# GAMES-UChile/mogptk

Hardware: AMD Instinct MI355X
Metric: log-marginal-likelihood+grad evals/sec, MOSM C=4 N=8192; 1/2/4/8 GPU (higher is better)
Workload: dtype f64

## Files before the change

mogptk_amd/csrc/flow.hip:

```cpp
#include "mogp_model.h"
#include <unistd.h>
#include <chrono>
#include <set>

#include <cstdio>
#include <cstdlib>

namespace mogp {

typedef double d4_t __attribute__((ext_vector_type(4)));
typedef double d2_t __attribute__((ext_vector_type(2)));

#define FL_BK 16
#define FL_ROWK 18
#define FL_WTM 4
#define FL_WTN 2
#define FL_NWJ 4
#define FL_NWI 2
#define FL_NT 512
#define FL_COLK (MOGP_TILE + 16)
#define FL_OPER (MOGP_TILE * FL_ROWK)
#define FL_LDS_DOUBLES (2 * 2 * FL_OPER)
#define FL_LDS_BYTES (FL_LDS_DOUBLES * 8 + 16 + 3 * 64 * 4 + 16)
static_assert(MOGP_TILE * FL_ROWK == 16 * FL_COLK, "one LDS operand slot serves both layouts");

#define FL_LDS_BARRIER() asm volatile("s_waitcnt lgkmcnt(0)\n\ts_barrier" ::: "memory")

template <int AKM, int BKM, bool MARK = false>
__device__ __forceinline__ void flow_tile(const double* Ap, const double* Bp, double* Cp, const int64_t ld, const int kt, const bool fresh,
                                          const double alpha, double* gemm_lds, unsigned long long* tr, unsigned* prog, double* const* Cpp, const double* alphap) {
    constexpr int WTM = FL_WTM, WTN = FL_WTN, NWJ = FL_NWJ, NWI = FL_NWI, NT = FL_NT;
    constexpr int TMR = MOGP_TILE, TNC = MOGP_TILE, COLK_A = FL_COLK, COLK_B = FL_COLK, OPER_A = FL_OPER, OPER_B = FL_OPER;
    constexpr int EPT_A = TMR * FL_BK / NT, EPT_B = TNC * FL_BK / NT;
    constexpr int NQ_A = EPT_A / 2, NQ_B = EPT_B / 2, TPR_A = FL_BK / EPT_A, TPR_B = FL_BK / EPT_B, TPK = NT / FL_BK;
    int tl = threadIdx.x;
    asm volatile("" : "+v"(tl));
    const int ln = tl & 63, wv = tl >> 6, wi = wv / NWJ, wj = wv % NWJ;
    const int64_t a_g = AKM ? (int64_t)(tl / TPK) * ld + (tl % TPK) * EPT_A : (int64_t)(tl / TPR_A) * ld + (tl % TPR_A) * EPT_A;
    const int64_t b_g = BKM ? (int64_t)(tl / TPK) * ld + (tl % TPK) * EPT_B : (int64_t)(tl / TPR_B) * ld + (tl % TPR_B) * EPT_B;
    const int a_l = AKM ? (tl / TPK) * COLK_A + (tl % TPK) * EPT_A : (tl / TPR_A) * FL_ROWK + (tl % TPR_A) * EPT_A;
    const int b_l = BKM ? (tl / TPK) * COLK_B + (tl % TPK) * EPT_B : (tl / TPR_B) * FL_ROWK + (tl % TPR_B) * EPT_B;
    const int64_t a_step = AKM ? (int64_t)FL_BK * ld : FL_BK;
    const int64_t b_step = BKM ? (int64_t)FL_BK * ld : FL_BK;
    const int crow = wi * (TMR / NWI) + (ln >> 4), ccol = wj * (TNC / NWJ) + (ln & 15);
    const int fa = AKM ? (ln >> 4) * COLK_A + wi * (TMR / NWI) + (ln & 15) : (wi * (TMR / NWI) + (ln & 15)) * FL_ROWK + (ln >> 4);
    const int fb = BKM ? (ln >> 4) * COLK_B + wj * (TNC / NWJ) + (ln & 15) : (wj * (TNC / NWJ) + (ln & 15)) * FL_ROWK + (ln >> 4);
    constexpr int fa_m = AKM ? 16 : 16 * FL_ROWK, fa_k = AKM ? 4 * COLK_A : 4;
    constexpr int fb_n = BKM ? 16 : 16 * FL_ROWK, fb_k = BKM ? 4 * COLK_B : 4;

    d4_t acc[WTM][WTN];
    if (!fresh) {
#pragma unroll
        for (int m = 0; m < WTM; ++m)
#pragma unroll
            for (int n = 0; n < WTN; ++n)
#pragma unroll
                for (int r = 0; r < 4; ++r) acc[m][n][r] = alpha * Cp[(int64_t)(crow + m * 16 + 4 * r) * ld + ccol + n * 16];
    } else {
#pragma unroll
        for (int m = 0; m < WTM; ++m)
#pragma unroll
            for (int n = 0; n < WTN; ++n) acc[m][n] = (d4_t){0.0, 0.0, 0.0, 0.0};
    }
    d2_t ra[NQ_A], rb[NQ_B];
    auto load_block = [&](int kb) {
        const d2_t* pa = reinterpret_cast<const d2_t*>(Ap + a_g + (int64_t)kb * a_step);
        const d2_t* pb = reinterpret_cast<const d2_t*>(Bp + b_g + (int64_t)kb * b_step);
#pragma unroll
        for (int q = 0; q < NQ_A; ++q) ra[q] = pa[q];
#pragma unroll
        for (int q = 0; q < NQ_B; ++q) rb[q] = pb[q];
    };
    auto write_block = [&](int buf) {
        double* sa = gemm_lds + buf * (OPER_A + OPER_B);
        double* sb = sa + OPER_A;
#pragma unroll
        for (int q = 0; q < NQ_A; ++q) *reinterpret_cast<d2_t*>(sa + a_l + 2 * q) = ra[q];
#pragma unroll
        for (int q = 0; q < NQ_B; ++q) *reinterpret_cast<d2_t*>(sb + b_l + 2 * q) = rb[q];
    };
    auto read_frag = [&](double (&av)[WTM], double (&bv)[WTN], int buf, int k4) {
        const double* sa = gemm_lds + buf * (OPER_A + OPER_B);
        const double* sb = sa + OPER_A;
#pragma unroll
        for (int m = 0; m < WTM; ++m) av[m] = sa[fa + m * fa_m + k4 * fa_k];
#pragma unroll
        for (int n = 0; n < WTN; ++n) bv[n] = sb[fb + n * fb_n + k4 * fb_k];
    };
    auto mma = [&](const double (&av)[WTM], const double (&bv)[WTN]) {
#pragma unroll
        for (int m = 0; m < WTM; ++m)
#pragma unroll
            for (int n = 0; n < WTN; ++n)
                acc[m][n] = __builtin_amdgcn_mfma_f64_16x16x4f64(av[m], bv[n], acc[m][n], 0, 0, 0);
    };
#define FL_MARK(v) do { if constexpr (MARK) { if (prog && ln == 0) { const unsigned v__ = (v); prog[wv] = v__; \
        if (wv == 0) { const unsigned kb__ = v__ & 0xffffu, now__ = (unsigned)(wall_clock64() >> 4); \
            if (v__ == 0x10000u) prog[8] = now__; else if (v__ == 0x30000u) prog[13] = now__; else if (v__ == 0x40000u) prog[14] = now__; \
            else if ((v__ >> 16) == 2u && (kb__ & 7u) == 0u) prog[9 + (kb__ >> 3)] = now__; } } } } while (0)
    FL_MARK(0x10000u);
    load_block(0);
    write_block(0);
    load_block(min(1, kt - 1));
    FL_LDS_BARRIER();
    if constexpr (MARK) { if (tr) tr[2] = wall_clock64(); }
    {
        double a0[WTM], b0[WTN], a1[WTM], b1[WTN];
        read_frag(a0, b0, 0, 0);
        for (int kb = 0; kb < kt; ++kb) {
            const int buf = kb & 1;
            read_frag(a1, b1, buf, 1);
            __builtin_amdgcn_sched_barrier(0);
            mma(a0, b0);
            __builtin_amdgcn_sched_barrier(0);
            read_frag(a0, b0, buf, 2);
            __builtin_amdgcn_sched_barrier(0);
            mma(a1, b1);
            __builtin_amdgcn_sched_barrier(0);
            write_block(buf ^ 1);
            FL_MARK(0x20000u + (unsigned)kb);
            load_block(min(kb + 2, kt - 1));
            read_frag(a1, b1, buf, 3);
            __builtin_amdgcn_sched_barrier(0);
            mma(a0, b0);
            __builtin_amdgcn_sched_barrier(0);
            FL_LDS_BARRIER();
            read_frag(a0, b0, buf ^ 1, 0);
            __builtin_amdgcn_sched_barrier(0);
            mma(a1, b1);
            __builtin_amdgcn_sched_barrier(0);
        }
    }
    FL_MARK(0x30000u);
    if constexpr (MARK) { if (tr) tr[3] = wall_clock64(); }
    int t2 = threadIdx.x;
    asm volatile("" : "+v"(t2));
    const int ln2 = t2 & 63, wv2 = t2 >> 6;
    const int crow2 = (wv2 / NWJ) * (TMR / NWI) + (ln2 >> 4), ccol2 = (wv2 % NWJ) * (TNC / NWJ) + (ln2 & 15);
    double* Cq = *Cpp;
    const double alpha2 = *alphap;
#pragma unroll
    for (int m = 0; m < WTM; ++m)
#pragma unroll
        for (int n = 0; n < WTN; ++n)
#pragma unroll
            for (int r = 0; r < 4; ++r)
                __hip_atomic_store(Cq + (int64_t)(crow2 + m * 16 + 4 * r) * ld + ccol2 + n * 16, alpha2 * acc[m][n][r], __ATOMIC_RELAXED,
                                   __HIP_MEMORY_SCOPE_AGENT);
    FL_MARK(0x40000u);
#undef FL_MARK
}

struct FlowArgs {
    double* bA; double* bL; double* bWt; double* bWm; double* bB;
    int64_t ld;
    const FlowTask* tasks;
    const int* qmeta;
    unsigned* flags;
    int nq, ncas, base_heads, base_err;
    unsigned nap_max;
    unsigned nap_calm;
    int nhi;
    int claim_one;
    int refill;
    const double* vy; double* vz; double* vzz; double* vpart;
    int64_t npad;
    unsigned long long* info;
    int post_base;
    unsigned char* done;
    unsigned* post;
    unsigned* diag;
    unsigned long long* trace;
};

struct FlowHot {
    double* bA; double* bL; double* bWt; double* bWm; double* bB; int64_t ld;
    const FlowTask* tasks; const int* qmeta; unsigned* flags;
    int nq, ncas, base_heads, base_err;
    unsigned nap_max, nap_calm;
};

__device__ __forceinline__ void flow_zrow(const FlowArgs& g, const int i, double* lds) {
    int tid = threadIdx.x;
    asm volatile("" : "+v"(tid));
    const int lane = tid & 63, wave = tid >> 6;
    const int K = (i + 1) * MOGP_TILE;
    const double* Wr = g.bWm + (int64_t)(i * MOGP_TILE + wave * 16) * g.ld + 2 * lane;
    const double* yp = g.vy + 2 * lane;
    double zsq = 0.0;
    for (int r4 = 0; r4 < 16; r4 += 4) {
        const double* p0 = Wr + (int64_t)r4 * g.ld;
        d2_t a0 = (d2_t){0.0, 0.0}, a1 = a0, a2 = a0, a3 = a0;
#pragma unroll 2
        for (int k = 0; k < K; k += MOGP_TILE) {
            const d2_t yv = *reinterpret_cast<const d2_t*>(yp + k);
            const d2_t w0 = *reinterpret_cast<const d2_t*>(p0 + k);
            const d2_t w1 = *reinterpret_cast<const d2_t*>(p0 + g.ld + k);
            const d2_t w2 = *reinterpret_cast<const d2_t*>(p0 + 2 * g.ld + k);
            const d2_t w3 = *reinterpret_cast<const d2_t*>(p0 + 3 * g.ld + k);
            a0 += w0 * yv; a1 += w1 * yv; a2 += w2 * yv; a3 += w3 * yv;
        }
        double s[4] = {a0[0] + a0[1], a1[0] + a1[1], a2[0] + a2[1], a3[0] + a3[1]};
#pragma unroll
        for (int u = 0; u < 4; ++u) {
#pragma unroll
            for (int off = 32; off > 0; off >>= 1) s[u] += __shfl_down(s[u], off, 64);
            if (lane == 0) {
                __hip_atomic_store(g.vz + (int64_t)i * MOGP_TILE + wave * 16 + r4 + u, s[u], __ATOMIC_RELAXED, __HIP_MEMORY_SCOPE_AGENT);
                zsq += s[u] * s[u];
            }
        }
    }
    if (lane == 0) lds[wave] = zsq;
    __syncthreads();
    if (tid == 0) {
        double t = 0.0;
        for (int w = 0; w < FL_NT / 64; ++w) t += lds[w];
        __hip_atomic_store(g.vzz + i, t, __ATOMIC_RELAXED, __HIP_MEMORY_SCOPE_AGENT);
    }
}
__device__ __forceinline__ void flow_apart(const FlowArgs& g, const int r0, const int nrows, const int rblk, const int jg, double* lds) {
    int tid = threadIdx.x;
    asm volatile("" : "+v"(tid));
    if (tid < nrows) lds[tid] = g.vz[r0 + tid];
    __syncthreads();
    const int64_t col = (int64_t)jg * FL_NT + tid;
    if (col < g.npad) {
        const double* Wc = g.bWm + (int64_t)r0 * g.ld + col;
        double a[4] = {0.0, 0.0, 0.0, 0.0};
#pragma unroll 2
        for (int r = 0; r < nrows; r += 4) {
#pragma unroll
            for (int u = 0; u < 4; ++u) a[u] = fma(Wc[(int64_t)(r + u) * g.ld], lds[r + u], a[u]);
        }
        __hip_atomic_store(g.vpart + (int64_t)rblk * g.npad + col, (a[0] + a[1]) + (a[2] + a[3]), __ATOMIC_RELAXED, __HIP_MEMORY_SCOPE_AGENT);
    }
}

#define FL_IDLE_LIMIT 4000u
#define FL_CALM_AFTER 48u
#define FL_DEEP_AFTER 128u
#define FL_DEEP_EVERY 32u
#define FL_LA 8

template <bool MARK>
__global__ __launch_bounds__(FL_NT, 4) void k_flow(const FlowArgs* __restrict__ gp, const FlowHot ha) {
    const FlowArgs& g = *gp;
    extern __shared__ __attribute__((aligned(16))) double gemm_lds[];
    int* pick = reinterpret_cast<int*>(gemm_lds + FL_LDS_DOUBLES);
    int* lst = pick + 4;
    double** ep_C = reinterpret_cast<double**>(lst + 192);
    double* ep_alpha = reinterpret_cast<double*>(lst + 194);
    if (threadIdx.x < 64) { lst[threadIdx.x] = -1; lst[64 + threadIdx.x] = -1; lst[128 + threadIdx.x] = 0; }
    for (;;) {
        int tid = threadIdx.x;
        asm volatile("" : "+v"(tid));
        const int wave = __builtin_amdgcn_readfirstlane(tid >> 6), lane = tid & 63;
        unsigned long long t_look = 0;
        if (MARK && g.trace && tid == 0) t_look = wall_clock64();
        if (MARK && g.post && tid == 0) {
            unsigned* po = g.post + (size_t)(g.post_base + blockIdx.x) * FLOW_POST_W;
            const unsigned now = (unsigned)(wall_clock64() >> 4);
            po[2] = 1u; po[4] = now;
            if (po[72] == 0u) { po[72] = now | 1u; po[74] = __builtin_amdgcn_s_getreg((31 << 11) | 4); po[75] = __builtin_amdgcn_s_getreg((3 << 11) | 20); }
        }
        if (wave == 0) {
            unsigned* heads = ha.flags + ha.base_heads;
            unsigned* err = ha.flags + ha.base_err;
            const int ncl = ha.ncas * FL_LA, nlanes = ncl + (ha.nq - ha.ncas);
            const bool is_cas = lane < ncl, is_eager = lane >= ncl && lane < nlanes;
            const int myq = is_cas ? lane / FL_LA : (is_eager ? ha.ncas + (lane - ncl) : 0), myk = is_cas ? lane % FL_LA : 0;
            int qbase = 0, qsize = 0;
            if (lane < nlanes) { qbase = ha.qmeta[2 * myq]; qsize = ha.qmeta[2 * myq + 1]; }
            int pend = lst[lane];
            int met_idx = lst[64 + lane], met_n = lst[128 + lane] & 0xff;
            bool exhausted = (lst[128 + lane] >> 8) != 0;
            unsigned long long cas_heads = 0;
            for (int q = 0; q < ha.ncas; ++q) cas_heads |= 1ull << (q * FL_LA);
            const unsigned long long eager_mask = nlanes >= 64 ? ~0ull << ncl : ((1ull << nlanes) - 1ull) & ~((1ull << ncl) - 1ull);
            unsigned idle = 0, naps = 0;
            int res = -1;
            unsigned nap = 0;
            for (;;) {
                int h = 0, idx = -1;
                const bool peek = is_eager && myq < g.nhi && pend < 0 && !exhausted;
                if (is_cas) {
                    h = (int)__hip_atomic_load(heads + myq, __ATOMIC_RELAXED, __HIP_MEMORY_SCOPE_AGENT);
                    h = __shfl(h, lane - myk, 64);
                    idx = h + myk < qsize ? h + myk : -1;
                } else if (peek) {
                    h = (int)__hip_atomic_load(heads + myq, __ATOMIC_RELAXED, __HIP_MEMORY_SCOPE_AGENT);
                    if (h >= qsize) exhausted = true; else idx = h;
                } else if (is_eager) {
                    idx = pend;
                }
                bool ready = false;
                const bool deep = idle >= FL_DEEP_AFTER && (idle & (FL_DEEP_EVERY - 1u)) == 0u;
                if (deep && is_cas) {
                    int h2 = (int)__hip_atomic_fetch_or(heads + myq, 0u, __ATOMIC_RELAXED, __HIP_MEMORY_SCOPE_AGENT);
                    h2 = __shfl(h2, lane - myk, 64);
                    if (h2 != h && myk == 0) __hip_atomic_fetch_add(g.diag + FLOW_DIAG_HEAD_STALE, 1u, __ATOMIC_RELAXED, __HIP_MEMORY_SCOPE_AGENT);
                    h = h2;
                    idx = h + myk < qsize ? h + myk : -1;
                }
                if (idx >= 0) {
                    const FlowTask* t = ha.tasks + qbase + idx;
                    const int nd = t->ndep;
                    if (idx != met_idx) { met_idx = idx; met_n = 0; }
                    ready = true;
                    int lead = met_n;
                    for (int d = 0; d < 4; ++d)
                        if (d >= met_n && d < nd) {
                            if (__hip_atomic_load(ha.flags + t->dep[d], __ATOMIC_RELAXED, __HIP_MEMORY_SCOPE_AGENT) < (unsigned)t->need[d]) ready = false;
                            else if (lead == d) lead = d + 1;
                        }
                    met_n = lead;
                    if (deep && !ready) {
                        bool ready2 = true;
                        unsigned seen = 0, which = 0;
                        for (int d = 0; d < 4; ++d)
                            if (d < nd) {
                                const unsigned v = __hip_atomic_fetch_or(ha.flags + t->dep[d], 0u, __ATOMIC_RELAXED, __HIP_MEMORY_SCOPE_AGENT);
                                if (v < (unsigned)t->need[d]) ready2 = false; else { seen = v; which = t->dep[d]; }
                            }
                        if (ready2) {
                            __hip_atomic_fetch_add(g.diag + FLOW_DIAG_DEP_STALE, 1u, __ATOMIC_RELAXED, __HIP_MEMORY_SCOPE_AGENT);
                            __hip_atomic_store(g.diag + FLOW_DIAG_LAST, which, __ATOMIC_RELAXED, __HIP_MEMORY_SCOPE_AGENT);
                            __hip_atomic_store(g.diag + FLOW_DIAG_LAST + 1, seen, __ATOMIC_RELAXED, __HIP_MEMORY_SCOPE_AGENT);
                            __hip_atomic_store(g.diag + FLOW_DIAG_LAST + 2, (unsigned)blockIdx.x | ((unsigned)__builtin_amdgcn_s_getreg((3 << 11) | 20) << 16), __ATOMIC_RELAXED, __HIP_MEMORY_SCOPE_AGENT);
                            ready = true;
                        }
                    }
                }
                if (deep && lane == 0) __hip_atomic_fetch_add(g.diag + FLOW_DIAG_DEEP, 1u, __ATOMIC_RELAXED, __HIP_MEMORY_SCOPE_AGENT);
                const unsigned long long mready = __ballot(ready);
                if (MARK && g.post) {
                    if (lane == 0) { g.post[(size_t)(g.post_base + blockIdx.x) * FLOW_POST_W + 6] = (unsigned)mready; g.post[(size_t)(g.post_base + blockIdx.x) * FLOW_POST_W + 7] = (unsigned)(mready >> 32); }
                    if (__hip_atomic_load(err, __ATOMIC_RELAXED, __HIP_MEMORY_SCOPE_AGENT) != 0u) { res = -3; break; }
                }
                const unsigned long long cand = mready & (cas_heads | eager_mask);
                if (cand) {
                    const int wl = __ffsll((long long)cand) - 1;
                    int ok = 0;
                    if (lane == wl) {
                        if (is_cas) {
                            unsigned cur = (unsigned)h;
                            for (;;) {
                                unsigned expect = cur;
                                if (__hip_atomic_compare_exchange_strong(heads + myq, &expect, cur + 1u, __ATOMIC_RELAXED, __ATOMIC_RELAXED,
                                                                         __HIP_MEMORY_SCOPE_AGENT)) { ok = 1; res = qbase + (int)cur; break; }
                                cur = expect;
                                const unsigned off = cur - (unsigned)h;
                                if (off >= FL_LA || !((mready >> (lane + off)) & 1ull)) break;
                            }
                        } else if (peek) {
                            const unsigned hh = __hip_atomic_fetch_add(heads + myq, 1u, __ATOMIC_RELAXED, __HIP_MEMORY_SCOPE_AGENT);
                            if (hh == (unsigned)h) { ok = 1; res = qbase + h; }
                            else if (hh < (unsigned)qsize) { pend = (int)hh; if (MARK && g.trace) g.trace[FLOW_TRACE_W * (size_t)(qbase + (int)hh) + 5] = (1ull << 63) | blockIdx.x; }
                            else exhausted = true;
                        } else {
                            ok = 1; res = qbase + pend;
                            if (g.refill && pend + 2 * (int)gridDim.x < qsize) {
                                const unsigned hh = __hip_atomic_fetch_add(heads + myq, 1u, __ATOMIC_RELAXED, __HIP_MEMORY_SCOPE_AGENT);
                                if (hh < (unsigned)qsize) { pend = (int)hh; if (MARK && g.trace) g.trace[FLOW_TRACE_W * (size_t)(qbase + (int)hh) + 5] = (1ull << 63) | blockIdx.x; } else { pend = -1; exhausted = true; }
                            } else pend = -1;
                        }
                    }
                    ok = __shfl(ok, wl, 64);
                    res = __shfl(res, wl, 64);
                    if (ok) break;
                    continue;
                }
                bool took = false;
                bool want = is_eager && myq >= g.nhi && pend < 0 && !exhausted;
                if (g.claim_one) {
                    const unsigned long long mw = __ballot(want);
                    want = want && mw && lane == __ffsll((long long)mw) - 1;
                }
                if (want) {
                    const unsigned hh = __hip_atomic_fetch_add(heads + myq, 1u, __ATOMIC_RELAXED, __HIP_MEMORY_SCOPE_AGENT);
                    if (hh < (unsigned)qsize) { pend = (int)hh; took = true; if (MARK && g.trace) g.trace[FLOW_TRACE_W * (size_t)(qbase + (int)hh) + 5] = (1ull << 63) | blockIdx.x; } else exhausted = true;
                }
                const bool open = is_cas ? (myk == 0 && h < qsize) : (is_eager && (pend >= 0 || !exhausted));
                if (!__ballot(open)) { res = -2; break; }
                if (__ballot(took)) continue;
                const unsigned cap = idle >= FL_CALM_AFTER ? ha.nap_calm : ha.nap_max;
                nap = nap < cap ? nap + 1u : cap;
                for (unsigned z = 0; z < (1u << nap); ++z) __builtin_amdgcn_s_sleep(32);
                ++naps;
                if ((++idle & 15u) == 0u) {
                    if (__hip_atomic_load(err, __ATOMIC_RELAXED, __HIP_MEMORY_SCOPE_AGENT) != 0u) { res = -3; break; }
                    if (idle > FL_IDLE_LIMIT) {
                        __hip_atomic_store(err, 0x700u, __ATOMIC_RELAXED, __HIP_MEMORY_SCOPE_AGENT);
                        res = -3;
                        break;
                    }
                }
            }
            lst[lane] = pend; lst[64 + lane] = met_idx; lst[128 + lane] = met_n | (exhausted ? 0x100 : 0);
            if (lane == 0) {
                pick[0] = res;
                pick[1] = (int)naps;
                if (res >= 0) __builtin_amdgcn_fence(__ATOMIC_ACQUIRE, "agent");
            }
            if (MARK && g.post && res < 0) {
                unsigned* po = g.post + (size_t)(g.post_base + blockIdx.x) * FLOW_POST_W;
                po[8 + lane] = is_eager ? (unsigned)(pend + 1) : 0u;
                if (lane == 0) { po[0] = (unsigned)(res + 4); po[1] = idle; po[2] = 3u; po[5] = (unsigned)(wall_clock64() >> 4); }
            }
        }
        __syncthreads();
        const int ti = __builtin_amdgcn_readfirstlane(pick[0]);
        if (ti < 0) {
            if (ti == -3 && tid == 0) atomicMin(g.info, (unsigned long long)MOGP_INFO_CHAIN_TIMEOUT);
            break;
        }
        const FlowTask* tp = ha.tasks + ti;
        const int var = tp->var, kt = tp->kt;
        const int ab = tp->abuf, bb = tp->bbuf, cb = tp->cbuf;
        const double* Ab = ab == 0 ? ha.bA : ab == 1 ? ha.bL : ab == 2 ? ha.bWt : ab == 3 ? ha.bWm : ha.bB;
        const double* Bb = bb == 0 ? ha.bA : bb == 1 ? ha.bL : bb == 2 ? ha.bWt : bb == 3 ? ha.bWm : ha.bB;
        double* Cb = cb == 0 ? ha.bA : cb == 1 ? ha.bL : cb == 2 ? ha.bWt : cb == 3 ? ha.bWm : ha.bB;
        const double* Ap = Ab + ((int64_t)tp->ar * ha.ld + tp->ac) * MOGP_TILE;
        const double* Bp = Bb + ((int64_t)tp->br * ha.ld + tp->bc) * MOGP_TILE;
        double* Cp = Cb + ((int64_t)tp->cr * ha.ld + tp->cc) * MOGP_TILE;
        const bool fresh = (var & 4) != 0;
        const double alpha = (var & 8) ? -1.0 : 1.0;
        unsigned long long* tr = (MARK && g.trace && tid == 0) ? g.trace + FLOW_TRACE_W * (size_t)ti : nullptr;
        if (tr) { tr[0] = t_look; tr[1] = wall_clock64(); }
        unsigned* prog = (MARK && g.post) ? g.post + (size_t)(g.post_base + blockIdx.x) * FLOW_POST_W + 80 : nullptr;
        if (MARK && g.post && tid == 0) {
            unsigned* po = g.post + (size_t)(g.post_base + blockIdx.x) * FLOW_POST_W;
            po[2] = 2u; po[3] = (unsigned)ti; po[73] += 1u; po[76] = (unsigned)(wall_clock64() >> 4);
        }
        if (var & 32) {
            if (g.vy) {
                if (var & 1) flow_apart(g, tp->ar * MOGP_TILE, kt * MOGP_TILE, tp->br, tp->ac, gemm_lds);
                else flow_zrow(g, tp->ar, gemm_lds);
            }
        } else {
        if (var & 16) __builtin_amdgcn_s_setprio(2);
        if (tid == 0) { *ep_C = Cp; *ep_alpha = alpha; }
        switch (var & 3) {
            case 0: flow_tile<0, 0, MARK>(Ap, Bp, Cp, ha.ld, kt, fresh, alpha, gemm_lds, tr, prog, ep_C, ep_alpha); break;
            case 1: flow_tile<0, 1, MARK>(Ap, Bp, Cp, ha.ld, kt, fresh, alpha, gemm_lds, tr, prog, ep_C, ep_alpha); break;
            default: flow_tile<1, 1, MARK>(Ap, Bp, Cp, ha.ld, kt, fresh, alpha, gemm_lds, tr, prog, ep_C, ep_alpha); break;
        }
        if (var & 16) __builtin_amdgcn_s_setprio(0);
        }
        asm volatile("s_waitcnt vmcnt(0)" ::: "memory");
        __syncthreads();
        if (tid == 0) {
            const unsigned s0 = tp->sig[0], s1 = tp->sig[1];
            if (s0 != FLOW_NOSIG) __hip_atomic_fetch_add(ha.flags + s0, 1u, __ATOMIC_RELAXED, __HIP_MEMORY_SCOPE_AGENT);
            if (s1 != FLOW_NOSIG) __hip_atomic_fetch_add(ha.flags + s1, 1u, __ATOMIC_RELAXED, __HIP_MEMORY_SCOPE_AGENT);
            if (MARK && g.done) g.done[ti] = 1;
            if (MARK && g.post) g.post[(size_t)(g.post_base + blockIdx.x) * FLOW_POST_W + 77] = (unsigned)(wall_clock64() >> 4);
            if (tr) {
                tr[4] = wall_clock64();
                tr[5] = ((unsigned long long)(unsigned)pick[1] << 32) | ((unsigned long long)__builtin_amdgcn_s_getreg((3 << 11) | 20) << 16) | blockIdx.x;
            }
        }
    }
}


namespace {
enum { PH_INTO = 0, PH_CHAIN = 600, PH_T6 = 601, PH_PANEL = 602, PH_UPDATE = 603, PH_T9 = 604, PH_ZROW = 605, PH_APART = 606, PH_XS = 607, PH_TU = 608 };
enum { Q_LOOK2 = 0, Q_INVCRIT = 1, Q_SEMI = 2 };
enum { BUF_A = 0, BUF_L = 1, BUF_WT = 2, BUF_WM = 3, BUF_B = 4 };
}

void flow_build(int nb, int ob, FlowPlan& p, int rhs_nt, bool replay) {
    p = FlowPlan();
    p.nb = nb; p.ob = ob; p.rhs_nt = rhs_nt; p.replay = replay;
    const int no = (nb + ob - 1) / ob;
    p.nouter = no;
    const uint32_t base_S = 0, base_R = base_S + (uint32_t)nb * nb, base_DG = base_R + (uint32_t)nb * no, base_PN = base_DG + no,
                   base_CH = base_PN + (uint32_t)no * nb, base_WT = base_CH + no, base_WC = base_WT + (uint32_t)nb * nb,
                   base_WF = base_WC + (uint32_t)no * nb, base_KV = base_WF + (uint32_t)no * nb, base_WR = base_KV + (uint32_t)nb * nb,
                   base_ZR = base_WR + no, base_TS = base_ZR + no, base_TR = base_TS + (uint32_t)rhs_nt * nb, base_XN = base_TR + (uint32_t)rhs_nt * no,
                   base_end = base_XN + (uint32_t)no * rhs_nt;
    p.base_heads = (int)base_end; p.base_err = p.base_heads + FLOW_MAXQ; p.nflags = p.base_err + 1;
    auto S = [&](int i, int j) { return base_S + (uint32_t)i * nb + j; };
    auto R = [&](int i, int c) { return base_R + (uint32_t)i * no + c; };
    auto DG = [&](int c) { return base_DG + (uint32_t)c; };
    auto PN = [&](int b, int i) { return base_PN + (uint32_t)b * nb + i; };
    auto CH = [&](int b) { return base_CH + (uint32_t)b; };
    auto WT = [&](int i, int j) { return base_WT + (uint32_t)i * nb + j; };
    auto WC = [&](int r, int j) { return base_WC + (uint32_t)r * nb + j; };
    auto WF = [&](int b, int j) { return base_WF + (uint32_t)b * nb + j; };
    auto KV = [&](int i, int j) { return base_KV + (uint32_t)i * nb + j; };
    auto WR = [&](int b) { return base_WR + (uint32_t)b; };
    auto ZR = [&](int b) { return base_ZR + (uint32_t)b; };
    auto TS = [&](int i, int j) { return base_TS + (uint32_t)i * nb + j; };
    auto TR = [&](int i, int c) { return base_TR + (uint32_t)i * no + c; };
    auto XN = [&](int b, int i) { return base_XN + (uint32_t)b * rhs_nt + i; };
    auto k0 = [&](int b) { return b * ob; };
    auto k1 = [&](int b) { return std::min(nb, (b + 1) * ob); };
    auto nk = [&](int b) { return k1(b) - k0(b); };
    auto blk = [&](int i) { return i / ob; };
    auto chain_wgs = [&](int b) { return nk(b) > 1 ? 13u : 2u; };

    std::vector<FlowTask> q[3], acc, vec;
    std::vector<std::vector<FlowTask>> into(no), trail(no);
    auto mk = [&](int b, int phase, int var, int kt) {
        FlowTask t{};
        t.var = (uint8_t)var; t.kt = (uint16_t)kt; t.ndep = 0; t.sig[0] = t.sig[1] = FLOW_NOSIG; t.key = (uint32_t)(b * FLOW_KEY_STEP + phase);
        return t;
    };
    auto dep = [&](FlowTask& t, uint32_t idx, unsigned need) {
        if (need == 0) return;
        t.dep[t.ndep] = idx; t.need[t.ndep] = (uint16_t)need; ++t.ndep;
    };
    auto opA = [](FlowTask& t, int buf, int r, int c) { t.abuf = (uint8_t)buf; t.ar = (uint16_t)r; t.ac = (uint16_t)c; };
    auto opB = [](FlowTask& t, int buf, int r, int c) { t.bbuf = (uint8_t)buf; t.br = (uint16_t)r; t.bc = (uint16_t)c; };
    auto opC = [](FlowTask& t, int buf, int r, int c) { t.cbuf = (uint8_t)buf; t.cr = (uint16_t)r; t.cc = (uint16_t)c; };
    const int KB = MOGP_TILE / FL_BK;
    double tiles_k = 0.0;

    auto crit_row = [&](int b, int i) { return !replay && i >= k1(b) && i < std::min(nb, k1(b) + ob); };
    auto pn_need = [&](int b, int i) { return (unsigned)((crit_row(b, i) ? 2 : 1) * nk(b)); };
    auto panel = [&](int b, int i, int c, bool prio) {
        FlowTask t = mk(b, PH_PANEL, 0 | 4 | (prio ? 16 : 0), KB * (c + 1));
        opA(t, BUF_A, i, k0(b)); opB(t, BUF_WM, k0(b) + c, k0(b)); opC(t, BUF_L, i, k0(b) + c);
        dep(t, CH(b), chain_wgs(b));
        dep(t, R(i, b), (unsigned)(nk(b) * b));
        t.sig[0] = PN(b, i);
        tiles_k += t.kt;
        return t;
    };
    auto update = [&](int b, int i, int j, bool prio) {
        FlowTask t = mk(b, PH_UPDATE, 0 | 8 | (prio ? 16 : 0), KB * nk(b));
        opA(t, BUF_L, i, k0(b)); opB(t, BUF_L, j, k0(b)); opC(t, BUF_A, i, j);
        dep(t, PN(b, i), pn_need(b, i));
        if (j != i) dep(t, PN(b, j), pn_need(b, j));
        dep(t, S(i, j), (unsigned)b);
        t.sig[0] = S(i, j);
        t.sig[1] = blk(i) == blk(j) ? DG(blk(j)) : R(i, blk(j));
        tiles_k += t.kt;
        return t;
    };
    auto t7 = [&](int b, int i, int c) {
        FlowTask t = mk(blk(i), PH_INTO + 2 * b, 1 | 4 | 8, KB * (nk(b) - c));
        opA(t, BUF_L, i, k0(b) + c); opB(t, BUF_WM, k0(b) + c, k0(b) + c); opC(t, BUF_WT, i, k0(b) + c);
        dep(t, PN(b, i), pn_need(b, i));
        t.sig[0] = WT(i, k0(b) + c); t.sig[1] = WC(blk(i), k0(b) + c);
        tiles_k += t.kt;
        return t;
    };
    auto t8 = [&](int b, int i, int j) {
        FlowTask t = mk(blk(i), PH_INTO + 2 * b + 1, 1 | 8, KB * nk(b));
        opA(t, BUF_L, i, k0(b)); opB(t, BUF_WM, k0(b), j); opC(t, BUF_WT, i, j);
        dep(t, PN(b, i), pn_need(b, i));
        dep(t, WF(b, j), (unsigned)nk(b));
        dep(t, WT(i, j), (unsigned)(b - blk(j)));
        t.sig[0] = WT(i, j); t.sig[1] = WC(blk(i), j);
        tiles_k += t.kt;
        return t;
    };
    auto t6 = [&](int b, int ti, int j) {
        FlowTask t = mk(b, PH_T6, 1 | 4, KB * (ti + 1));
        opA(t, BUF_WM, k0(b) + ti, k0(b)); opB(t, BUF_WT, k0(b), j); opC(t, BUF_WM, k0(b) + ti, j);
        dep(t, CH(b), chain_wgs(b));
        dep(t, WC(b, j), (unsigned)(nk(b) * (b - blk(j))));
        t.sig[0] = WF(b, j); t.sig[1] = WR(b);
        tiles_k += t.kt;
        return t;
    };
    static const bool t9_full = std::getenv("MOGP_FLOW_T9FULL") && std::atoi(std::getenv("MOGP_FLOW_T9FULL")) != 0;
    auto t9 = [&](int b, int i, int j) {
        const int r0 = (i >= k0(b) && !t9_full) ? i : k0(b);
        FlowTask t = mk(b, PH_T9, 2 | (i >= k0(b) ? 4 : 0), KB * (k1(b) - r0));
        opA(t, BUF_WM, r0, i); opB(t, BUF_WM, r0, j); opC(t, BUF_B, i, j);
        bool ch = false;
        if (i >= k0(b)) { dep(t, CH(b), chain_wgs(b)); ch = true; } else dep(t, WF(b, i), (unsigned)nk(b));
        if (j != i) { if (j >= k0(b)) { if (!ch) dep(t, CH(b), chain_wgs(b)); } else dep(t, WF(b, j), (unsigned)nk(b)); }
        dep(t, KV(i, j), (unsigned)(b - blk(i)));
        t.sig[0] = KV(i, j);
        tiles_k += t.kt;
        return t;
    };

    auto xs = [&](int b, int i, int c) {
        FlowTask t = mk(b, PH_XS, 0 | 4, KB * (c + 1));
        opA(t, BUF_WT, i, k0(b)); opB(t, BUF_WM, k0(b) + c, k0(b)); opC(t, BUF_B, i, k0(b) + c);
        dep(t, CH(b), chain_wgs(b));
        dep(t, TR(i, b), (unsigned)(nk(b) * b));
        t.sig[0] = XN(b, i);
        tiles_k += t.kt;
        return t;
    };
    auto tu = [&](int b, int i, int j) {
        FlowTask t = mk(b, PH_TU, 0 | 8, KB * nk(b));
        opA(t, BUF_B, i, k0(b)); opB(t, BUF_L, j, k0(b)); opC(t, BUF_WT, i, j);
        dep(t, XN(b, i), (unsigned)nk(b));
        dep(t, PN(b, j), pn_need(b, j));
        dep(t, TS(i, j), (unsigned)b);
        t.sig[0] = TS(i, j); t.sig[1] = TR(i, blk(j));
        tiles_k += t.kt;
        return t;
    };
    std::vector<FlowTask> rrest;

    p.chain.resize(no);
    for (int b = 0; b < no; ++b) {
        const int a0 = k1(b), a1 = std::min(nb, a0 + ob), a2 = std::min(nb, a1 + ob);
        FlowPlan::Chain& c = p.chain[b];
        c = FlowPlan::Chain{};
        c.done_idx = CH(b); c.expect = chain_wgs(b);
        c.t1_nwait = 0;
        for (int i = a0; i < a1 && b > 0; ++i) { c.t1_widx[c.t1_nwait] = R(i, b); c.t1_wval[c.t1_nwait] = (uint32_t)(nk(b) * b); ++c.t1_nwait; }
        c.t1_sig_base = PN(b, a0); c.t1_sig_per_row = 2u * (uint32_t)nk(b);
        if (a1 > a0) { const int n1 = a1 - a0; c.t2_widx = DG(b + 1); c.t2_wval = (uint32_t)(n1 * (n1 + 1) / 2 * b); }
        if (replay) {
            for (int i = a0; i < a1; ++i) for (int cc = 0; cc < nk(b); ++cc) q[Q_LOOK2].push_back(panel(b, i, cc, true));
            for (int i = a0; i < a1; ++i) for (int j = a0; j <= i; ++j) q[Q_LOOK2].push_back(update(b, i, j, true));
        }
        for (int i = a1; i < a2; ++i) for (int cc = 0; cc < nk(b); ++cc) q[Q_LOOK2].push_back(panel(b, i, cc, true));
        for (int i = a1; i < a2; ++i) for (int j = a0; j < a1; ++j) q[Q_LOOK2].push_back(update(b, i, j, true));
        for (int i = a1; i < a2; ++i) for (int j = a1; j <= i; ++j) q[Q_LOOK2].push_back(update(b, i, j, true));
        for (int i = a2; i < nb; ++i) for (int cc = 0; cc < nk(b); ++cc) q[Q_SEMI].push_back(panel(b, i, cc, false));
        for (int i = a2; i < nb; ++i) for (int j = a0; j < a2; ++j) q[Q_SEMI].push_back(update(b, i, j, false));
        for (int i = a2; i < nb; ++i) for (int j = a2; j <= i; ++j) trail[b].push_back(update(b, i, j, false));
        if (rhs_nt > 0) {
            for (int i = 0; i < rhs_nt; ++i) for (int cc = 0; cc < nk(b); ++cc) q[Q_INVCRIT].push_back(xs(b, i, cc));
            for (int i = 0; i < rhs_nt; ++i) for (int j = a0; j < a1; ++j) q[Q_INVCRIT].push_back(tu(b, i, j));
            for (int i = 0; i < rhs_nt; ++i) for (int j = a1; j < nb; ++j) rrest.push_back(tu(b, i, j));
            continue;
        }
        for (int j = 0; j < k0(b); ++j) for (int ti = 0; ti < nk(b); ++ti) q[Q_INVCRIT].push_back(t6(b, ti, j));
        for (int i = a0; i < a1; ++i) for (int cc = 0; cc < nk(b); ++cc) q[Q_INVCRIT].push_back(t7(b, i, cc));
        for (int i = a0; i < a1; ++i) for (int j = 0; j < k0(b); ++j) q[Q_INVCRIT].push_back(t8(b, i, j));
        for (int bs = 0; bs + 2 <= b; ++bs) {
            for (int i = k0(b); i < k1(b); ++i) for (int cc = 0; cc < nk(bs); ++cc) into[b].push_back(t7(bs, i, cc));
            for (int i = k0(b); i < k1(b); ++i) for (int j = 0; j < k0(bs); ++j) into[b].push_back(t8(bs, i, j));
        }
        for (int i = 0; i < k1(b); ++i) for (int j = 0; j <= i; ++j) acc.push_back(t9(b, i, j));
        for (int i = k0(b); i < k1(b); ++i) {
            FlowTask t = mk(b, PH_ZROW, 32, 1);
            t.ar = (uint16_t)i;
            dep(t, CH(b), chain_wgs(b));
            dep(t, WR(b), (unsigned)(nk(b) * k0(b)));
            t.sig[0] = ZR(b);
            vec.push_back(t);
        }
        for (int jg = 0; jg * 4 < k1(b); ++jg) {
            FlowTask t = mk(b, PH_APART, 32 | 1, nk(b));
            t.ar = (uint16_t)k0(b); t.br = (uint16_t)b; t.ac = (uint16_t)jg;
            dep(t, ZR(b), (unsigned)nk(b));
            vec.push_back(t);
        }
    }
    std::vector<const std::vector<FlowTask>*> order = {&q[Q_LOOK2], &q[Q_SEMI], &q[Q_INVCRIT], &vec};
    for (int d = 2; d < no + 3; ++d) {
        if (d < no && !into[d].empty()) order.push_back(&into[d]);
        if (d - 3 >= 0 && d - 3 < no && !trail[d - 3].empty()) order.push_back(&trail[d - 3]);
    }
    order.push_back(rhs_nt > 0 ? &rrest : &acc);
    for (size_t k = order.size(); k-- > 1;) if (order[k]->empty()) order.erase(order.begin() + (long)k);
    if ((int)order.size() > FLOW_MAXQ) {
        std::vector<FlowTask> rest;
        std::vector<const std::vector<FlowTask>*> tail(order.begin() + (FLOW_MAXQ - 2), order.end() - 1);
        for (auto* v : tail) rest.insert(rest.end(), v->begin(), v->end());
        std::stable_sort(rest.begin(), rest.end(), [](const FlowTask& x, const FlowTask& y) { return x.key < y.key; });
        p.folded = rest;
        order.erase(order.begin() + (FLOW_MAXQ - 2), order.end() - 1);
        order.insert(order.end() - 1, &p.folded);
    }
    p.nq = (int)order.size();
    for (int qi = 0; qi < p.nq; ++qi) {
        p.qbase[qi] = (int)p.tasks.size(); p.qsize[qi] = (int)order[qi]->size();
        p.tasks.insert(p.tasks.end(), order[qi]->begin(), order[qi]->end());
    }
    p.flops = 2.0 * MOGP_TILE * MOGP_TILE * FL_BK * tiles_k;
}

__global__ void k_alpha_sum(const double* __restrict__ part, int64_t npad, int no, int ob, double* __restrict__ out) {
    const int64_t col = (int64_t)blockIdx.x * blockDim.x + threadIdx.x;
    if (col >= npad) return;
    double s = 0.0;
    for (int r = (int)(col / MOGP_TILE) / ob; r < no; ++r) s += part[(int64_t)r * npad + col];
    out[col] = s;
}
int launch_flow_alpha_sum(const Spd& w, double* alpha, hipStream_t st) {
    const FlowPlan& p = w.flow_cur ? *w.flow_cur : w.flow;
    hipLaunchKernelGGL(k_alpha_sum, dim3((unsigned)((w.Npad + 255) / 256)), dim3(256), 0, st, w.vec_part, w.Npad, p.nouter, p.ob, alpha);
    HIP_TRY(hipGetLastError());
    return 0;
}

bool flow_enabled(const mogp_model* m, const Spd& w) {
    const char* eo = std::getenv("MOGP_FLOW");
    const char* en = std::getenv("MOGP_FLOW_MIN");
    const int on = eo ? std::atoi(eo) : 1, nmin = en ? std::atoi(en) : 8;
    if (!on || (m->no_flow && m->n_fact < m->flow_retry_at) || !chain_enabled(m) || !m->ctx->st_priv) return false;
    if (m->kinv_sparse && &w == &m->k) return false;
    return w.nb >= nmin && w.nb <= 0xfff0;
}

int spd_potri_flow(mogp_model* m, Spd& w, const FlowRhs* rhs) {
    const int nb = w.nb, ob = 4;
    const int64_t ld = w.Npad;
    int rc;
    const auto host_t0 = std::chrono::steady_clock::now();
    hipStream_t crit = m->st, priv = m->st_priv, bulk = m->st2;
    if (w.Wm.n < (size_t)ld * ld) {
        if ((rc = w.Wm.ensure((size_t)ld * ld))) return rc;
        HIP_TRY(hipMemsetAsync(w.Wm.p, 0, (size_t)ld * ld * sizeof(double), crit));
    }
    if ((rc = w.Lm.ensure((size_t)ld * ld))) return rc;
    if (!rhs && (rc = w.Wt.ensure((size_t)ld * ld))) return rc;
    const bool replay = m->replay_flow && !rhs && &w == &m->k;
    FlowPlan& plan = rhs ? w.flow_rhs : replay ? w.flow_replay : w.flow;
    DevBuf<FlowTask>& d_tasks = rhs ? w.flow_tasks_rhs : replay ? w.flow_tasks_replay : w.flow_tasks;
    DevBuf<int>& d_qmeta = rhs ? w.flow_qmeta_rhs : replay ? w.flow_qmeta_replay : w.flow_qmeta;
    const int rhs_nt = rhs ? rhs->nt : 0;
    if (plan.nb != nb || plan.ob != ob || plan.rhs_nt != rhs_nt) {
        flow_build(nb, ob, plan, rhs_nt, replay);
        if ((rc = d_tasks.ensure(plan.tasks.size()))) return rc;
        if ((rc = d_qmeta.ensure(2 * FLOW_MAXQ))) return rc;
        int qm[2 * FLOW_MAXQ] = {0};
        for (int q = 0; q < plan.nq; ++q) { qm[2 * q] = plan.qbase[q]; qm[2 * q + 1] = plan.qsize[q]; }
        HIP_TRY(hipStreamSynchronize(crit));
        HIP_TRY(dev_upload(d_tasks.p, plan.tasks.data(), plan.tasks.size() * sizeof(FlowTask)));
        HIP_TRY(dev_upload(d_qmeta.p, qm, sizeof(qm)));
    }
    if ((rc = w.flow_flags.ensure((size_t)plan.nflags))) return rc;
    if (!w.flow_diag.p) {
        if ((rc = w.flow_diag.ensure(FLOW_DIAG_WORDS))) return rc;
        HIP_TRY(hipMemsetAsync(w.flow_diag.p, 0, FLOW_DIAG_WORDS * sizeof(unsigned), crit));
    }
    w.flow_cur = &plan;
    const FlowPlan& p = plan;
    const int nouter = p.nouter;
    if ((rc = w.chain_flags.ensure((size_t)(nouter + 1) * MOGP_CHAIN_FLAGS))) return rc;
    HIP_TRY(hipMemsetAsync(w.chain_flags.p, 0, (size_t)(nouter + 1) * MOGP_CHAIN_FLAGS * sizeof(unsigned), crit));
    HIP_TRY(hipMemsetAsync(w.flow_flags.p, 0, (size_t)p.nflags * sizeof(unsigned), crit));
    if (replay) {
        std::vector<unsigned> preset((size_t)p.nflags, 0u);
        for (const FlowPlan::Chain& c : p.chain) preset[c.done_idx] = c.expect;
        HIP_TRY(hipMemcpyAsync(w.flow_flags.p, preset.data(), preset.size() * sizeof(unsigned), hipMemcpyHostToDevice, crit));
        HIP_TRY(hipStreamSynchronize(crit));
    }
    if (!rhs && w.want_vec && w.vec_zz) HIP_TRY(hipMemsetAsync(w.vec_zz, 0, (size_t)((ld + 3) / 4) * sizeof(double), crit));
    static const bool want_trace = std::getenv("MOGP_FLOW_TRACE") && std::atoi(std::getenv("MOGP_FLOW_TRACE")) != 0;
    if (want_trace) {
        if ((rc = w.flow_trace.ensure(FLOW_TRACE_W * p.tasks.size() + 4 * (size_t)nouter))) return rc;
        HIP_TRY(hipMemsetAsync(w.flow_trace.p, 0, w.flow_trace.n * sizeof(unsigned long long), crit));
    }
    while ((int)w.inv_ev.size() < 4) {
        hipEvent_t e;
        HIP_TRY(hipEventCreateWithFlags(&e, hipEventDisableTiming));
        w.inv_ev.push_back(e);
    }
    hipEvent_t start = w.inv_ev[0], e_flow = w.inv_ev[1], e_chain = w.inv_ev[2];
    HIP_TRY(hipEventRecord(start, crit));
    HIP_TRY(hipStreamWaitEvent(bulk, start, 0));
    HIP_TRY(hipStreamWaitEvent(priv, start, 0));

    static std::atomic<unsigned long long> attr_done{0ull};
    static std::atomic<unsigned long long> attr_done_dbg{0ull};
    { int r__ = set_max_dynamic_lds(reinterpret_cast<const void*>(k_flow<false>), FL_LDS_BYTES, attr_done); if (r__) return r__; }
    { int r__ = set_max_dynamic_lds(reinterpret_cast<const void*>(k_flow<true>), FL_LDS_BYTES, attr_done_dbg); if (r__) return r__; }
    static const int wg_per_cu = std::getenv("MOGP_FLOW_WGS") ? std::max(1, std::atoi(std::getenv("MOGP_FLOW_WGS"))) : 2;
    int cus = (m->ctx->ncu > 0 ? m->ctx->ncu : 256) - m->ctx->ncu_reserved;
    { static const int drop = std::getenv("MOGP_FLOW_DROP_CUS") ? std::atoi(std::getenv("MOGP_FLOW_DROP_CUS")) : 16;
// ... 339 lines not shown
```

Measured before the change: 95.37.

## Cache task descriptors in LDS/registers and prefetch C tile before first block write

```diff
diff --git a/mogptk_amd/csrc/flow.hip b/mogptk_amd/csrc/flow.hip
--- a/mogptk_amd/csrc/flow.hip
+++ b/mogptk_amd/csrc/flow.hip
@@ -21,7 +21,8 @@
 #define FL_COLK (MOGP_TILE + 16)
 #define FL_OPER (MOGP_TILE * FL_ROWK)
 #define FL_LDS_DOUBLES (2 * 2 * FL_OPER)
-#define FL_LDS_BYTES (FL_LDS_DOUBLES * 8 + 16 + 3 * 64 * 4 + 16)
+#define FL_LDS_BYTES (FL_LDS_DOUBLES * 8 + 16 + 3 * 64 * 4 + 2 * 64 * 4 + 4 * 64 * 16 + 64 + 16)
+static_assert(2 * FL_LDS_BYTES <= 160 * 1024, "two workgroups of k_flow per CU");
 static_assert(MOGP_TILE * FL_ROWK == 16 * FL_COLK, "one LDS operand slot serves both layouts");
 
 #define FL_LDS_BARRIER() asm volatile("s_waitcnt lgkmcnt(0)\n\ts_barrier" ::: "memory")
@@ -49,19 +50,6 @@
     constexpr int fb_n = BKM ? 16 : 16 * FL_ROWK, fb_k = BKM ? 4 * COLK_B : 4;
 
     d4_t acc[WTM][WTN];
-    if (!fresh) {
-#pragma unroll
-        for (int m = 0; m < WTM; ++m)
-#pragma unroll
-            for (int n = 0; n < WTN; ++n)
-#pragma unroll
-                for (int r = 0; r < 4; ++r) acc[m][n][r] = alpha * Cp[(int64_t)(crow + m * 16 + 4 * r) * ld + ccol + n * 16];
-    } else {
-#pragma unroll
-        for (int m = 0; m < WTM; ++m)
-#pragma unroll
-            for (int n = 0; n < WTN; ++n) acc[m][n] = (d4_t){0.0, 0.0, 0.0, 0.0};
-    }
     d2_t ra[NQ_A], rb[NQ_B];
     auto load_block = [&](int kb) {
         const d2_t* pa = reinterpret_cast<const d2_t*>(Ap + a_g + (int64_t)kb * a_step);
@@ -100,8 +88,33 @@
             else if ((v__ >> 16) == 2u && (kb__ & 7u) == 0u) prog[9 + (kb__ >> 3)] = now__; } } } } while (0)
     FL_MARK(0x10000u);
     load_block(0);
+    __builtin_amdgcn_sched_barrier(0);
+    if (!fresh) {
+#pragma unroll
+        for (int m = 0; m < WTM; ++m)
+#pragma unroll
+            for (int n = 0; n < WTN; ++n)
+#pragma unroll
+                for (int r = 0; r < 4; ++r) acc[m][n][r] = Cp[(int64_t)(crow + m * 16 + 4 * r) * ld + ccol + n * 16];
+    } else {
+#pragma unroll
+        for (int m = 0; m < WTM; ++m)
+#pragma unroll
+            for (int n = 0; n < WTN; ++n) acc[m][n] = (d4_t){0.0, 0.0, 0.0, 0.0};
+    }
+    __builtin_amdgcn_sched_barrier(0);
     write_block(0);
+    __builtin_amdgcn_sched_barrier(0);
     load_block(min(1, kt - 1));
+    __builtin_amdgcn_sched_barrier(0);
+    if (!fresh) {
+#pragma unroll
+        for (int m = 0; m < WTM; ++m)
+#pragma unroll
+            for (int n = 0; n < WTN; ++n)
+#pragma unroll
+                for (int r = 0; r < 4; ++r) acc[m][n][r] = alpha * acc[m][n][r];
+    }
     FL_LDS_BARRIER();
     if constexpr (MARK) { if (tr) tr[2] = wall_clock64(); }
     {
@@ -249,9 +262,19 @@
     extern __shared__ __attribute__((aligned(16))) double gemm_lds[];
     int* pick = reinterpret_cast<int*>(gemm_lds + FL_LDS_DOUBLES);
     int* lst = pick + 4;
-    double** ep_C = reinterpret_cast<double**>(lst + 192);
-    double* ep_alpha = reinterpret_cast<double*>(lst + 194);
-    if (threadIdx.x < 64) { lst[threadIdx.x] = -1; lst[64 + threadIdx.x] = -1; lst[128 + threadIdx.x] = 0; }
+    int* qm = lst + 192;
+    uint4* dsc = reinterpret_cast<uint4*>(qm + 128);
+    unsigned* tsk = reinterpret_cast<unsigned*>(dsc + 256);
+    double** ep_C = reinterpret_cast<double**>(tsk + 16);
+    double* ep_alpha = reinterpret_cast<double*>(tsk + 18);
+    if (threadIdx.x < 64) {
+        const int lane0 = threadIdx.x, ncl0 = ha.ncas * FL_LA, nl0 = ncl0 + (ha.nq - ha.ncas);
+        const int q0 = lane0 < ncl0 ? lane0 / FL_LA : (lane0 < nl0 ? ha.ncas + (lane0 - ncl0) : 0);
+        lst[lane0] = -1; lst[64 + lane0] = -1; lst[128 + lane0] = 0;
+        qm[lane0] = lane0 < nl0 ? ha.qmeta[2 * q0] : 0; qm[64 + lane0] = lane0 < nl0 ? ha.qmeta[2 * q0 + 1] : 0;
+#pragma unroll
+        for (int j = 0; j < 4; ++j) dsc[64 * j + lane0] = make_uint4(0u, 0u, 0u, 0u);
+    }
     for (;;) {
         int tid = threadIdx.x;
         asm volatile("" : "+v"(tid));
@@ -270,11 +293,16 @@
             const int ncl = ha.ncas * FL_LA, nlanes = ncl + (ha.nq - ha.ncas);
             const bool is_cas = lane < ncl, is_eager = lane >= ncl && lane < nlanes;
             const int myq = is_cas ? lane / FL_LA : (is_eager ? ha.ncas + (lane - ncl) : 0), myk = is_cas ? lane % FL_LA : 0;
-            int qbase = 0, qsize = 0;
-            if (lane < nlanes) { qbase = ha.qmeta[2 * myq]; qsize = ha.qmeta[2 * myq + 1]; }
+            const int qbase = qm[lane], qsize = qm[64 + lane];
             int pend = lst[lane];
-            int met_idx = lst[64 + lane], met_n = lst[128 + lane] & 0xff;
+            int cur = lst[64 + lane], met_n = lst[128 + lane] & 0xff;
             bool exhausted = (lst[128 + lane] >> 8) != 0;
+            uint4 d0 = dsc[lane], d1 = dsc[64 + lane], d2 = dsc[128 + lane], d3 = dsc[192 + lane];
+            auto fetch_desc = [&](int i) {
+                const uint4* t4 = reinterpret_cast<const uint4*>(ha.tasks + qbase + i);
+                d0 = t4[0]; d1 = t4[1]; d2 = t4[2]; d3 = t4[3];
+                cur = i; met_n = 0;
+            };
             unsigned long long cas_heads = 0;
             for (int q = 0; q < ha.ncas; ++q) cas_heads |= 1ull << (q * FL_LA);
             const unsigned long long eager_mask = nlanes >= 64 ? ~0ull << ncl : ((1ull << nlanes) - 1ull) & ~((1ull << ncl) - 1ull);
@@ -284,12 +312,19 @@
             for (;;) {
                 int h = 0, idx = -1;
                 const bool peek = is_eager && myq < g.nhi && pend < 0 && !exhausted;
+                unsigned cv[4] = {~0u, ~0u, ~0u, ~0u};
+                if (is_cas || peek) h = (int)__hip_atomic_load(heads + myq, __ATOMIC_RELAXED, __HIP_MEMORY_SCOPE_AGENT);
+                if (cur >= 0) {
+                    const unsigned dp[4] = {d1.y, d1.z, d1.w, d2.x};
+                    const int nd = (int)(d1.x >> 16);
+#pragma unroll
+                    for (int d = 0; d < 4; ++d)
+                        if (d >= met_n && d < nd) cv[d] = __hip_atomic_load(ha.flags + dp[d], __ATOMIC_RELAXED, __HIP_MEMORY_SCOPE_AGENT);
+                }
                 if (is_cas) {
-                    h = (int)__hip_atomic_load(heads + myq, __ATOMIC_RELAXED, __HIP_MEMORY_SCOPE_AGENT);
                     h = __shfl(h, lane - myk, 64);
                     idx = h + myk < qsize ? h + myk : -1;
                 } else if (peek) {
-                    h = (int)__hip_atomic_load(heads + myq, __ATOMIC_RELAXED, __HIP_MEMORY_SCOPE_AGENT);
                     if (h >= qsize) exhausted = true; else idx = h;
                 } else if (is_eager) {
                     idx = pend;
@@ -303,25 +338,37 @@
                     h = h2;
                     idx = h + myk < qsize ? h + myk : -1;
                 }
+                const bool fresh_task = idx >= 0 && idx != cur;
+                if (__ballot(fresh_task)) {
+                    if (fresh_task) fetch_desc(idx);
+                    if (fresh_task) {
+                        const unsigned dp[4] = {d1.y, d1.z, d1.w, d2.x};
+                        const int nd = (int)(d1.x >> 16);
+#pragma unroll
+                        for (int d = 0; d < 4; ++d) cv[d] = d < nd ? __hip_atomic_load(ha.flags + dp[d], __ATOMIC_RELAXED, __HIP_MEMORY_SCOPE_AGENT) : ~0u;
+                    }
+                }
                 if (idx >= 0) {
-                    const FlowTask* t = ha.tasks + qbase + idx;
-                    const int nd = t->ndep;
-                    if (idx != met_idx) { met_idx = idx; met_n = 0; }
+                    const unsigned dp[4] = {d1.y, d1.z, d1.w, d2.x};
+                    const unsigned nee[4] = {d2.y & 0xffffu, d2.y >> 16, d2.z & 0xffffu, d2.z >> 16};
+                    const int nd = (int)(d1.x >> 16);
                     ready = true;
                     int lead = met_n;
+#pragma unroll
                     for (int d = 0; d < 4; ++d)
                         if (d >= met_n && d < nd) {
-                            if (__hip_atomic_load(ha.flags + t->dep[d], __ATOMIC_RELAXED, __HIP_MEMORY_SCOPE_AGENT) < (unsigned)t->need[d]) ready = false;
+                            if (cv[d] < nee[d]) ready = false;
                             else if (lead == d) lead = d + 1;
                         }
                     met_n = lead;
                     if (deep && !ready) {
                         bool ready2 = true;
                         unsigned seen = 0, which = 0;
+#pragma unroll
                         for (int d = 0; d < 4; ++d)
                             if (d < nd) {
-                                const unsigned v = __hip_atomic_fetch_or(ha.flags + t->dep[d], 0u, __ATOMIC_RELAXED, __HIP_MEMORY_SCOPE_AGENT);
-                                if (v < (unsigned)t->need[d]) ready2 = false; else { seen = v; which = t->dep[d]; }
+                                const unsigned v = __hip_atomic_fetch_or(ha.flags + dp[d], 0u, __ATOMIC_RELAXED, __HIP_MEMORY_SCOPE_AGENT);
+                                if (v < nee[d]) ready2 = false; else { seen = v; which = dp[d]; }
                             }
                         if (ready2) {
                             __hip_atomic_fetch_add(g.diag + FLOW_DIAG_DEP_STALE, 1u, __ATOMIC_RELAXED, __HIP_MEMORY_SCOPE_AGENT);
@@ -341,34 +388,45 @@
                 const unsigned long long cand = mready & (cas_heads | eager_mask);
                 if (cand) {
                     const int wl = __ffsll((long long)cand) - 1;
-                    int ok = 0;
+                    int ok = 0, own = lane;
+                    bool refill_now = false;
                     if (lane == wl) {
                         if (is_cas) {
-                            unsigned cur = (unsigned)h;
+                            unsigned cur_h = (unsigned)h;
                             for (;;) {
-                                unsigned expect = cur;
-                                if (__hip_atomic_compare_exchange_strong(heads + myq, &expect, cur + 1u, __ATOMIC_RELAXED, __ATOMIC_RELAXED,
-                                                                         __HIP_MEMORY_SCOPE_AGENT)) { ok = 1; res = qbase + (int)cur; break; }
-                                cur = expect;
-                                const unsigned off = cur - (unsigned)h;
+                                unsigned expect = cur_h;
+                                if (__hip_atomic_compare_exchange_strong(heads + myq, &expect, cur_h + 1u, __ATOMIC_RELAXED, __ATOMIC_RELAXED,
+                                                                         __HIP_MEMORY_SCOPE_AGENT)) { ok = 1; res = qbase + (int)cur_h; own = lane + (int)(cur_h - (unsigned)h); break; }
+                                cur_h = expect;
+                                const unsigned off = cur_h - (unsigned)h;
                                 if (off >= FL_LA || !((mready >> (lane + off)) & 1ull)) break;
                             }
                         } else if (peek) {
                             const unsigned hh = __hip_atomic_fetch_add(heads + myq, 1u, __ATOMIC_RELAXED, __HIP_MEMORY_SCOPE_AGENT);
                             if (hh == (unsigned)h) { ok = 1; res = qbase + h; }
-                            else if (hh < (unsigned)qsize) { pend = (int)hh; if (MARK && g.trace) g.trace[FLOW_TRACE_W * (size_t)(qbase + (int)hh) + 5] = (1ull << 63) | blockIdx.x; }
+                            else if (hh < (unsigned)qsize) { pend = (int)hh; fetch_desc(pend); if (MARK && g.trace) g.trace[FLOW_TRACE_W * (size_t)(qbase + (int)hh) + 5] = (1ull << 63) | blockIdx.x; }
                             else exhausted = true;
                         } else {
                             ok = 1; res = qbase + pend;
-                            if (g.refill && pend + 2 * (int)gridDim.x < qsize) {
-                                const unsigned hh = __hip_atomic_fetch_add(heads + myq, 1u, __ATOMIC_RELAXED, __HIP_MEMORY_SCOPE_AGENT);
-                                if (hh < (unsigned)qsize) { pend = (int)hh; if (MARK && g.trace) g.trace[FLOW_TRACE_W * (size_t)(qbase + (int)hh) + 5] = (1ull << 63) | blockIdx.x; } else { pend = -1; exhausted = true; }
-                            } else pend = -1;
+                            refill_now = g.refill && pend + 2 * (int)gridDim.x < qsize;
+                            pend = -1;
                         }
                     }
                     ok = __shfl(ok, wl, 64);
                     res = __shfl(res, wl, 64);
-                    if (ok) break;
+                    own = __shfl(own, wl, 64);
+                    if (ok) {
+                        if (lane == own) {
+                            uint4* t4 = reinterpret_cast<uint4*>(tsk);
+                            t4[0] = d0; t4[1] = d1; t4[2] = d2; t4[3] = d3;
+                            if (!is_cas) cur = -1;
+                        }
+                        if (refill_now) {
+                            const unsigned hh = __hip_atomic_fetch_add(heads + myq, 1u, __ATOMIC_RELAXED, __HIP_MEMORY_SCOPE_AGENT);
+                            if (hh < (unsigned)qsize) { pend = (int)hh; fetch_desc(pend); if (MARK && g.trace) g.trace[FLOW_TRACE_W * (size_t)(qbase + (int)hh) + 5] = (1ull << 63) | blockIdx.x; } else exhausted = true;
+                        }
+                        break;
+                    }
                     continue;
                 }
                 bool took = false;
@@ -379,7 +437,7 @@
                 }
                 if (want) {
                     const unsigned hh = __hip_atomic_fetch_add(heads + myq, 1u, __ATOMIC_RELAXED, __HIP_MEMORY_SCOPE_AGENT);
-                    if (hh < (unsigned)qsize) { pend = (int)hh; took = true; if (MARK && g.trace) g.trace[FLOW_TRACE_W * (size_t)(qbase + (int)hh) + 5] = (1ull << 63) | blockIdx.x; } else exhausted = true;
+                    if (hh < (unsigned)qsize) { pend = (int)hh; took = true; fetch_desc(pend); if (MARK && g.trace) g.trace[FLOW_TRACE_W * (size_t)(qbase + (int)hh) + 5] = (1ull << 63) | blockIdx.x; } else exhausted = true;
                 }
                 const bool open = is_cas ? (myk == 0 && h < qsize) : (is_eager && (pend >= 0 || !exhausted));
                 if (!__ballot(open)) { res = -2; break; }
@@ -397,7 +455,8 @@
                     }
                 }
             }
-            lst[lane] = pend; lst[64 + lane] = met_idx; lst[128 + lane] = met_n | (exhausted ? 0x100 : 0);
+            lst[lane] = pend; lst[64 + lane] = cur; lst[128 + lane] = met_n | (exhausted ? 0x100 : 0);
+            dsc[lane] = d0; dsc[64 + lane] = d1; dsc[128 + lane] = d2; dsc[192 + lane] = d3;
             if (lane == 0) {
                 pick[0] = res;
                 pick[1] = (int)naps;
@@ -415,15 +474,17 @@
             if (ti == -3 && tid == 0) atomicMin(g.info, (unsigned long long)MOGP_INFO_CHAIN_TIMEOUT);
             break;
         }
-        const FlowTask* tp = ha.tasks + ti;
-        const int var = tp->var, kt = tp->kt;
-        const int ab = tp->abuf, bb = tp->bbuf, cb = tp->cbuf;
+        const unsigned w0 = __builtin_amdgcn_readfirstlane(tsk[0]), w1 = __builtin_amdgcn_readfirstlane(tsk[1]), w2 = __builtin_amdgcn_readfirstlane(tsk[2]),
+                       w3 = __builtin_amdgcn_readfirstlane(tsk[3]), w4 = __builtin_amdgcn_readfirstlane(tsk[4]);
+        const int var = (int)(w3 >> 24), kt = (int)(w4 & 0xffffu);
+        const int ab = (int)(w3 & 0xffu), bb = (int)((w3 >> 8) & 0xffu), cb = (int)((w3 >> 16) & 0xffu);
+        const int t_ar = (int)(w0 & 0xffffu), t_ac = (int)(w0 >> 16), t_br = (int)(w1 & 0xffffu), t_bc = (int)(w1 >> 16), t_cr = (int)(w2 & 0xffffu), t_cc = (int)(w2 >> 16);
         const double* Ab = ab == 0 ? ha.bA : ab == 1 ? ha.bL : ab == 2 ? ha.bWt : ab == 3 ? ha.bWm : ha.bB;
         const double* Bb = bb == 0 ? ha.bA : bb == 1 ? ha.bL : bb == 2 ? ha.bWt : bb == 3 ? ha.bWm : ha.bB;
         double* Cb = cb == 0 ? ha.bA : cb == 1 ? ha.bL : cb == 2 ? ha.bWt : cb == 3 ? ha.bWm : ha.bB;
-        const double* Ap = Ab + ((int64_t)tp->ar * ha.ld + tp->ac) * MOGP_TILE;
-        const double* Bp = Bb + ((int64_t)tp->br * ha.ld + tp->bc) * MOGP_TILE;
-        double* Cp = Cb + ((int64_t)tp->cr * ha.ld + tp->cc) * MOGP_TILE;
+        const double* Ap = Ab + ((int64_t)t_ar * ha.ld + t_ac) * MOGP_TILE;
+        const double* Bp = Bb + ((int64_t)t_br * ha.ld + t_bc) * MOGP_TILE;
+        double* Cp = Cb + ((int64_t)t_cr * ha.ld + t_cc) * MOGP_TILE;
         const bool fresh = (var & 4) != 0;
         const double alpha = (var & 8) ? -1.0 : 1.0;
         unsigned long long* tr = (MARK && g.trace && tid == 0) ? g.trace + FLOW_TRACE_W * (size_t)ti : nullptr;
@@ -435,8 +496,8 @@
         }
         if (var & 32) {
             if (g.vy) {
-                if (var & 1) flow_apart(g, tp->ar * MOGP_TILE, kt * MOGP_TILE, tp->br, tp->ac, gemm_lds);
-                else flow_zrow(g, tp->ar, gemm_lds);
+                if (var & 1) flow_apart(g, t_ar * MOGP_TILE, kt * MOGP_TILE, t_br, t_ac, gemm_lds);
+                else flow_zrow(g, t_ar, gemm_lds);
             }
         } else {
         if (var & 16) __builtin_amdgcn_s_setprio(2);
@@ -451,7 +512,7 @@
         asm volatile("s_waitcnt vmcnt(0)" ::: "memory");
         __syncthreads();
         if (tid == 0) {
-            const unsigned s0 = tp->sig[0], s1 = tp->sig[1];
+            const unsigned s0 = tsk[11], s1 = tsk[12];
             if (s0 != FLOW_NOSIG) __hip_atomic_fetch_add(ha.flags + s0, 1u, __ATOMIC_RELAXED, __HIP_MEMORY_SCOPE_AGENT);
             if (s1 != FLOW_NOSIG) __hip_atomic_fetch_add(ha.flags + s1, 1u, __ATOMIC_RELAXED, __HIP_MEMORY_SCOPE_AGENT);
             if (MARK && g.done) g.done[ti] = 1;
@@ -463,6 +524,9 @@
         }
     }
 }
+static_assert(offsetof(FlowTask, ar) == 0 && offsetof(FlowTask, br) == 4 && offsetof(FlowTask, cr) == 8 && offsetof(FlowTask, abuf) == 12 && offsetof(FlowTask, var) == 15 &&
+              offsetof(FlowTask, kt) == 16 && offsetof(FlowTask, ndep) == 18 && offsetof(FlowTask, dep) == 20 && offsetof(FlowTask, need) == 36 &&
+              offsetof(FlowTask, sig) == 44, "k_flow's view of FlowTask");
 
 
 namespace {
```

Result: no change. 95.41 (median of 2 runs) (+0.0%).
